# FyroxEngine/Fyrox

Measured on NVIDIA H100. Metric: nodes culled + verts skinned /sec, higher is better.
Workload: dtype f32

## Files before the change

fyrox_b200/csrc/fyx_kernels.cu:

```cuda
#include <cstdlib>
#include <cstring>

#include <cuda_fp16.h>

#include "fyx_internal.h"
#include "fyx_trs.cuh"

namespace fyx {

__device__ __forceinline__ float4 ld_stream(const float4 *p)
{
    float4 v;
    asm volatile("ld.global.nc.L1::no_allocate.v4.f32 {%0,%1,%2,%3}, [%4];"
                 : "=f"(v.x), "=f"(v.y), "=f"(v.z), "=f"(v.w)
                 : "l"(p));
    return v;
}
__device__ __forceinline__ float2 ld_stream(const float2 *p)
{
    float2 v;
    asm volatile("ld.global.nc.L1::no_allocate.v2.f32 {%0,%1}, [%2];" : "=f"(v.x), "=f"(v.y) : "l"(p));
    return v;
}
__device__ __forceinline__ uint4 ld_stream(const uint4 *p)
// ... 657 lines not shown
        bs_pre[r] = (b < b1) ? fa.bone_slot[b] : FYX_NONE;
        si_pre[r] = (b < b1 && fa.stale_idx) ? fa.stale_idx[b] : FYX_NONE;
    }
    const uint32_t nf = a.flags[slot];
    nf_out = nf;
    wx = a.wa[0][slot];
    wy = a.wa[1][slot];
    wz = a.wa[2][slot];
    if (!(nf & F_DIRTY)) return;
    float mnx = wx.x, mny = wy.x, mnz = wz.x, mxx = wx.y, mxy = wy.y, mxz = wz.y;
    uint32_t kmnx = 0, kmny = 0, kmnz = 0, kmxx = 0, kmxy = 0, kmxz = 0;
    auto add_bone = [&](const uint32_t b, const uint32_t bs, const uint32_t si) {
        if (bs == FYX_NONE) return;
        float px, py, pz;
        if (si != FYX_NONE) {
            const float4 o = fa.stale_pos[si];
            px = o.x; py = o.y; pz = o.z;
        } else {
            px = a.G[0][bs].w;
            py = a.G[1][bs].w;
            pz = a.G[2][bs].w;
        }
        const uint32_t key = b - b0 + 1u;
        if (px < mnx) { mnx = px; kmnx = key; }
        if (py < mny) { mny = py; kmny = key; }
        if (pz < mnz) { mnz = pz; kmnz = key; }
        if (px > mxx) { mxx = px; kmxx = key; }
        if (py > mxy) { mxy = py; kmxy = key; }
        if (pz > mxz) { mxz = pz; kmxz = key; }
    };
#pragma unroll
    for (int r = 0; r < 2; ++r) add_bone(b0 + lane + 32u * r, bs_pre[r], si_pre[r]);
    for (uint32_t b = b0 + lane + 64u; b < b1; b += 32)
        add_bone(b, fa.bone_slot[b], fa.stale_idx ? fa.stale_idx[b] : FYX_NONE);
#pragma unroll
    for (int o = 16; o > 0; o >>= 1) {
        fold_min(mnx, kmnx, __shfl_xor_sync(0xFFFFFFFFu, mnx, o), __shfl_xor_sync(0xFFFFFFFFu, kmnx, o));
        fold_min(mny, kmny, __shfl_xor_sync(0xFFFFFFFFu, mny, o), __shfl_xor_sync(0xFFFFFFFFu, kmny, o));
        fold_min(mnz, kmnz, __shfl_xor_sync(0xFFFFFFFFu, mnz, o), __shfl_xor_sync(0xFFFFFFFFu, kmnz, o));
        fold_max(mxx, kmxx, __shfl_xor_sync(0xFFFFFFFFu, mxx, o), __shfl_xor_sync(0xFFFFFFFFu, kmxx, o));
        fold_max(mxy, kmxy, __shfl_xor_sync(0xFFFFFFFFu, mxy, o), __shfl_xor_sync(0xFFFFFFFFu, kmxy, o));
        fold_max(mxz, kmxz, __shfl_xor_sync(0xFFFFFFFFu, mxz, o), __shfl_xor_sync(0xFFFFFFFFu, kmxz, o));
    }
    wx = make_float2(mnx, mxx);
    wy = make_float2(mny, mxy);
    wz = make_float2(mnz, mxz);
    if (lane == 0) {
        a.wa[0][slot] = wx;
        a.wa[1][slot] = wy;
        a.wa[2][slot] = wz;
    }
}

template <int NFT>
__global__ void __launch_bounds__(kBlock) k_fold_bones(const NodeArrays a, const FoldArrays fa, const CullParams cp)
{
    pdl_trigger();
    pdl_wait();
    constexpr int kWarps = kBlock / 32;
    __shared__ float2 s_box[3][kWarps];
    __shared__ uint32_t s_nf[kWarps];
    const uint32_t warp = threadIdx.x >> 5, lane = threadIdx.x & 31u;
    const uint32_t i = blockIdx.x * kWarps + warp;
    uint32_t nf = 0u;
    float2 wx = make_float2(0.f, 0.f), wy = wx, wz = wx;
    if (i < fa.n) fold_mesh(a, fa, i, lane, nf, wx, wy, wz);
    if (NFT < 0) return;
    if (lane == 0) {
        s_box[0][warp] = wx;
        s_box[1][warp] = wy;
        s_box[2][warp] = wz;
        s_nf[warp] = (i < fa.n) ? nf : 0u;
    }
    __syncthreads();
    if (warp != 0) return;
    uint32_t vis_bits = 0u, gi = 0u, slot = 0u;
    const uint32_t m = blockIdx.x * kWarps + lane;
    if (lane < kWarps && m < fa.n) {
        PackedConsts kc;
        kc.one = make_float2(cp.one, cp.one);
        kc.negzero = make_float2(cp.negzero, cp.negzero);
        slot = fa.node_slot[m];
        const float2 bx = s_box[0][lane], by = s_box[1][lane], bz = s_box[2][lane];
        vis_bits = cull_bits<(NFT > 0 ? NFT : 0)>(s_nf[lane], a.mask[slot], bx, by, bz, cp, kc, aabb_is_tame(bx, by, bz), 0xFFFFFFFFu);
        if (vis_bits) gi = a.gidx[slot];
    }
    compact_emit_warp(vis_bits, gi, slot, cp);
}

__global__ void __launch_bounds__(kBlock) k_snapshot_bones(const NodeArrays a, const uint32_t n_late, const uint32_t *late_slot,
                                                           float4 *stale_pos)
{
    const uint32_t e = blockIdx.x * kBlock + threadIdx.x;
    if (e >= n_late) return;
    const uint32_t s = late_slot[e];
    stale_pos[e] = make_float4(a.G[0][s].w, a.G[1][s].w, a.G[2][s].w, 0.0f);
}

__device__ __forceinline__ void palette_entry(const NodeArrays &a, const SkinArrays &sk, const uint32_t e)
{
    const uint32_t bs = sk.bone_slot[e];
    Affine P;
    if (bs != FYX_NONE) {
        Affine Gm, IB;
        Gm.r0 = a.G[0][bs];
        Gm.r1 = a.G[1][bs];
        Gm.r2 = a.G[2][bs];
        IB.r0 = ld_stream(sk.ib[0] + e);
        IB.r1 = ld_stream(sk.ib[1] + e);
        IB.r2 = ld_stream(sk.ib[2] + e);
        P = affine_mul(Gm, IB);
    } else {
        P = affine_identity();
    }
    float4 *o = reinterpret_cast<float4 *>(sk.palette + 16 * (size_t)e);
    o[0] = make_float4(P.r0.x, P.r1.x, P.r2.x, 0.0f);
    o[1] = make_float4(P.r0.y, P.r1.y, P.r2.y, 0.0f);
    o[2] = make_float4(P.r0.z, P.r1.z, P.r2.z, 0.0f);
    o[3] = make_float4(P.r0.w, P.r1.w, P.r2.w, 1.0f);
}

__global__ void __launch_bounds__(kBlock) k_palette(const NodeArrays a, const SkinArrays sk)
{
    pdl_trigger();
    pdl_wait();
    const uint32_t e = blockIdx.x * kBlock + threadIdx.x;
    if (e < sk.n_entries) palette_entry(a, sk, e);
}

__device__ __forceinline__ float2 lo2(const float4 v) { return make_float2(v.x, v.y); }
__device__ __forceinline__ float2 hi2(const float4 v) { return make_float2(v.z, v.w); }

template <int S, int LOG2C>
__device__ __forceinline__ void skin_fill_palette(float4 *s_pal, const float *palette, const uint32_t bone_off, const uint32_t n_bones)
{
    constexpr int C = 1 << LOG2C;
    constexpr int PL = S * C;
    for (uint32_t b = threadIdx.x; b < n_bones; b += kBlock) {
        const float4 *m = reinterpret_cast<const float4 *>(palette + 16 * (size_t)(bone_off + b));
        const float4 c0 = m[0], c1 = m[1], c2 = m[2], c3 = m[3];
        const float4 A = make_float4(c0.x, c0.y, c1.x, c1.y);
        const float4 B = make_float4(c2.x, c2.y, c3.x, c3.y);
        const float4 Z = make_float4(c0.z, c1.z, c2.z, c3.z);
#pragma unroll
        for (int c = 0; c < C; ++c) {
            s_pal[0 * PL + c * S + b] = A;
            s_pal[1 * PL + c * S + b] = B;
            s_pal[2 * PL + c * S + b] = Z;
        }
    }
}

template <int S, int LOG2C>
__device__ __forceinline__ void skin_quad(const float4 *s_pal, const uint32_t lane, const float4 x4, const float4 y4, const float4 z4,
                                          const float4 nx4, const float4 ny4, const float4 nz4, const float4 w0, const float4 w1,
                                          const float4 w2, const float4 w3, const uint4 iq, float4 *po, float4 *no,
                                          const PackedConsts kc)
{
    constexpr int C = 1 << LOG2C;
    constexpr int PL = S * C;
    const float px[4] = {x4.x, x4.y, x4.z, x4.w}, py[4] = {y4.x, y4.y, y4.z, y4.w}, pz[4] = {z4.x, z4.y, z4.z, z4.w};
    const float nx[4] = {nx4.x, nx4.y, nx4.z, nx4.w}, ny[4] = {ny4.x, ny4.y, ny4.z, ny4.w}, nz[4] = {nz4.x, nz4.y, nz4.z, nz4.w};
    const float wk4[4][4] = {{w0.x, w1.x, w2.x, w3.x}, {w0.y, w1.y, w2.y, w3.y}, {w0.z, w1.z, w2.z, w3.z}, {w0.w, w1.w, w2.w, w3.w}};
    const uint32_t iv[4] = {iq.x, iq.y, iq.z, iq.w};
    float ox[4], oy[4], oz[4], mx[4], my[4], mz[4];
#pragma unroll
    for (int v = 0; v < 4; ++v) {
        const float2 pxx = make_float2(px[v], px[v]), pyy = make_float2(py[v], py[v]), pzz = make_float2(pz[v], pz[v]);
        const float2 nxx = make_float2(nx[v], nx[v]), nyy = make_float2(ny[v], ny[v]), nzz = make_float2(nz[v], nz[v]);
        const float2 pnx = make_float2(px[v], nx[v]), pny = make_float2(py[v], ny[v]), pnz = make_float2(pz[v], nz[v]);
        float2 acc_p = make_float2(0.0f, 0.0f), acc_n = make_float2(0.0f, 0.0f), acc_z = make_float2(0.0f, 0.0f);
        const float *wk = wk4[v];
#pragma unroll
        for (int k = 0; k < 4; ++k) {
            const uint32_t bone = (iv[v] >> (8 * k)) & 0xFFu;
            const float4 *row = s_pal + (((lane - bone) & (uint32_t)(C - 1)) * S + bone);
            const float4 A = row[0], B = row[PL], Z = row[2 * PL];
            const float2 ww = make_float2(wk[k], wk[k]);
            const float2 t = add2(add2(add2(mul2(lo2(A), pxx, kc), mul2(hi2(A), pyy, kc), kc), mul2(lo2(B), pzz, kc), kc), hi2(B), kc);
            acc_p = add2(acc_p, mul2(t, ww, kc), kc);
            const float2 r = add2(add2(mul2(lo2(A), nxx, kc), mul2(hi2(A), nyy, kc), kc), mul2(lo2(B), nzz, kc), kc);
            acc_n = add2(acc_n, mul2(r, ww, kc), kc);
            float2 z = add2(add2(mul2(pnx, make_float2(Z.x, Z.x), kc), mul2(pny, make_float2(Z.y, Z.y), kc), kc), mul2(pnz, make_float2(Z.z, Z.z), kc), kc);
            z.x = FYX_ADD(z.x, Z.w);
            acc_z = add2(acc_z, mul2(z, ww, kc), kc);
        }
        ox[v] = acc_p.x; oy[v] = acc_p.y; oz[v] = acc_z.x;
        mx[v] = acc_n.x; my[v] = acc_n.y; mz[v] = acc_z.y;
    }
    st_stream(po + 0, make_float4(ox[0], oy[0], oz[0], ox[1]));
    st_stream(po + 1, make_float4(oy[1], oz[1], ox[2], oy[2]));
    st_stream(po + 2, make_float4(oz[2], ox[3], oy[3], oz[3]));
    st_stream(no + 0, make_float4(mx[0], my[0], mz[0], mx[1]));
    st_stream(no + 1, make_float4(my[1], mz[1], mx[2], my[2]));
    st_stream(no + 2, make_float4(mz[2], mx[3], my[3], mz[3]));
}

template <int S, int LOG2C>
__device__ __forceinline__ void skin_pair(const float4 *s_pal, const uint32_t lane, const float2 x2, const float2 y2, const float2 z2, const float2 nx2,
                                          const float2 ny2, const float2 nz2, const float2 w0, const float2 w1, const float2 w2, const float2 w3,
                                          const uint2 iq, float2 *po, float2 *no, const PackedConsts kc)
{
    constexpr int C = 1 << LOG2C;
    constexpr int PL = S * C;
    const float px[2] = {x2.x, x2.y}, py[2] = {y2.x, y2.y}, pz[2] = {z2.x, z2.y};
    const float nx[2] = {nx2.x, nx2.y}, ny[2] = {ny2.x, ny2.y}, nz[2] = {nz2.x, nz2.y};
    const float wk2[2][4] = {{w0.x, w1.x, w2.x, w3.x}, {w0.y, w1.y, w2.y, w3.y}};
    const uint32_t iv[2] = {iq.x, iq.y};
    float ox[2], oy[2], oz[2], mx[2], my[2], mz[2];
#pragma unroll
    for (int v = 0; v < 2; ++v) {
        const float2 pxx = make_float2(px[v], px[v]), pyy = make_float2(py[v], py[v]), pzz = make_float2(pz[v], pz[v]);
        const float2 nxx = make_float2(nx[v], nx[v]), nyy = make_float2(ny[v], ny[v]), nzz = make_float2(nz[v], nz[v]);
        const float2 pnx = make_float2(px[v], nx[v]), pny = make_float2(py[v], ny[v]), pnz = make_float2(pz[v], nz[v]);
        float2 acc_p = make_float2(0.0f, 0.0f), acc_n = make_float2(0.0f, 0.0f), acc_z = make_float2(0.0f, 0.0f);
        const float *wk = wk2[v];
#pragma unroll
        for (int k = 0; k < 4; ++k) {
            const uint32_t bone = (iv[v] >> (8 * k)) & 0xFFu;
            const float4 *row = s_pal + (((lane - bone) & (uint32_t)(C - 1)) * S + bone);
            const float4 A = row[0], B = row[PL], Z = row[2 * PL];
            const float2 ww = make_float2(wk[k], wk[k]);
            const float2 t = add2(add2(add2(mul2(lo2(A), pxx, kc), mul2(hi2(A), pyy, kc), kc), mul2(lo2(B), pzz, kc), kc), hi2(B), kc);
            acc_p = add2(acc_p, mul2(t, ww, kc), kc);
            const float2 r = add2(add2(mul2(lo2(A), nxx, kc), mul2(hi2(A), nyy, kc), kc), mul2(lo2(B), nzz, kc), kc);
            acc_n = add2(acc_n, mul2(r, ww, kc), kc);
            float2 z = add2(add2(mul2(pnx, make_float2(Z.x, Z.x), kc), mul2(pny, make_float2(Z.y, Z.y), kc), kc), mul2(pnz, make_float2(Z.z, Z.z), kc), kc);
            z.x = FYX_ADD(z.x, Z.w);
            acc_z = add2(acc_z, mul2(z, ww, kc), kc);
        }
        ox[v] = acc_p.x; oy[v] = acc_p.y; oz[v] = acc_z.x;
        mx[v] = acc_n.x; my[v] = acc_n.y; mz[v] = acc_z.y;
    }
    st_stream(po + 0, make_float2(ox[0], oy[0]));
    st_stream(po + 1, make_float2(oz[0], ox[1]));
    st_stream(po + 2, make_float2(oy[1], oz[1]));
    st_stream(no + 0, make_float2(mx[0], my[0]));
    st_stream(no + 1, make_float2(mz[0], mx[1]));
    st_stream(no + 2, make_float2(my[1], mz[1]));
}

template <int S, int LOG2C, int MINB>
__global__ void __launch_bounds__(kBlock, MINB) k_skin2(const SkinArrays sk, const SkinTile *__restrict__ tiles, const uint32_t n_tiles, const float one,
                                                      const float negzero)
{
    extern __shared__ float4 smem[];
    float4 *const s_pal = smem;
    PackedConsts kc;
    kc.one = make_float2(one, one);
    kc.negzero = make_float2(negzero, negzero);
    const SkinTile T = tiles[blockIdx.x];
    pdl_wait();
    skin_fill_palette<S, LOG2C>(s_pal, sk.palette, T.bone_off, T.n_bones);
    __syncthreads();
    const uint32_t lane = threadIdx.x & 31u;
    for (uint32_t h = threadIdx.x; h < 2u * T.n_quads; h += kBlock) {
        const size_t quad = (size_t)T.quad_start + (h >> 1);
        const float2 *row = reinterpret_cast<const float2 *>(sk.vblk + (quad >> 5) * kVblkStride + (quad & 31)) + (h & 1u);
        const float2 x2 = ld_stream(row + 0 * 64), y2 = ld_stream(row + 1 * 64), z2 = ld_stream(row + 2 * 64);
        const float2 nx2 = ld_stream(row + 3 * 64), ny2 = ld_stream(row + 4 * 64), nz2 = ld_stream(row + 5 * 64);
        const float2 w0 = ld_stream(row + 6 * 64), w1 = ld_stream(row + 7 * 64), w2 = ld_stream(row + 8 * 64), w3 = ld_stream(row + 9 * 64);
        const float2 iqf = ld_stream(row + 10 * 64);
        const uint2 iq = make_uint2(__float_as_uint(iqf.x), __float_as_uint(iqf.y));
        const size_t pair = 2 * quad + (h & 1u);
        skin_pair<S, LOG2C>(s_pal, lane, x2, y2, z2, nx2, ny2, nz2, w0, w1, w2, w3, iq, reinterpret_cast<float2 *>(sk.opos) + 3 * pair,
                            reinterpret_cast<float2 *>(sk.onrm) + 3 * pair, kc);
    }
}

__device__ __forceinline__ void bs_axpy(float4 &v, const uint2 h, const float w)
{
    const __half2 a = *reinterpret_cast<const __half2 *>(&h.x), b = *reinterpret_cast<const __half2 *>(&h.y);
    const float2 fa = __half22float2(a), fb = __half22float2(b);
    v.x = FYX_ADD(v.x, FYX_MUL(fa.x, w));
    v.y = FYX_ADD(v.y, FYX_MUL(fa.y, w));
    v.z = FYX_ADD(v.z, FYX_MUL(fb.x, w));
    v.w = FYX_ADD(v.w, FYX_MUL(fb.y, w));
}

__device__ __forceinline__ void apply_blend_shapes(const SkinArrays &sk, const SkinTile &T, const uint32_t q, float4 &x4, float4 &y4, float4 &z4,
                                                   float4 &nx4, float4 &ny4, float4 &nz4)
{
    const uint32_t e = T.local_quad0 + q;
    const uint2 *r0 = sk.bs + ((size_t)T.bs_off + (e >> 5)) * kBsBlockU2 + (e & 31u);
    const size_t shape_stride = (size_t)T.bs_blocks * kBsBlockU2;
    for (uint32_t sidx = 0; sidx < T.n_shapes; ++sidx) {
        const float w = sk.bs_w[T.w_off + sidx];
        const uint2 *r = r0 + sidx * shape_stride;
        const uint2 hx = r[0 * 32], hy = r[1 * 32], hz = r[2 * 32], hnx = r[3 * 32], hny = r[4 * 32], hnz = r[5 * 32];
        bs_axpy(x4, hx, w);
        bs_axpy(y4, hy, w);
        bs_axpy(z4, hz, w);
        bs_axpy(nx4, hnx, w);
        bs_axpy(ny4, hny, w);
        bs_axpy(nz4, hnz, w);
    }
}

__global__ void __launch_bounds__(kBlock) k_bs_layout(const uint32_t n_verts, const uint32_t n_shapes, const uint32_t layer_stride,
                                                      const uint16_t *rec, uint16_t *dst, const uint32_t bs_blocks)
{
    const uint64_t t = (uint64_t)blockIdx.x * kBlock + threadIdx.x;
    const uint64_t per_shape = (uint64_t)bs_blocks * 128;
    if (t >= per_shape * n_shapes) return;
    const uint32_t sidx = (uint32_t)(t / per_shape), v = (uint32_t)(t % per_shape);
    uint16_t h[6] = {0, 0, 0, 0, 0, 0};
    if (v < n_verts) {
        const uint16_t *r = rec + ((size_t)sidx * layer_stride + v) * 9;
        for (int k = 0; k < 6; ++k) h[k] = r[k];
    }
    uint16_t *blk = dst + ((size_t)sidx * bs_blocks + (v >> 7)) * (kBsBlockU2 * 4);
    const uint32_t g = (v >> 2) & 31u, j = v & 3u;
    for (int k = 0; k < 6; ++k) blk[(k * 32 + g) * 4 + j] = h[k];
}

void launch_bs_layout(cudaStream_t s, uint32_t n_verts, uint32_t n_shapes, uint32_t layer_stride, const uint16_t *d_records, uint2 *d_dst, uint32_t bs_blocks)
{
    if (!n_shapes || !bs_blocks) return;
    k_bs_layout<<<(unsigned)(((uint64_t)bs_blocks * 128 * n_shapes + kBlock - 1) / kBlock), kBlock, 0, s>>>(n_verts, n_shapes, layer_stride, d_records,
                                                                                                        reinterpret_cast<uint16_t *>(d_dst), bs_blocks);
}

template <int S, int LOG2C, int MINB, bool BS>
__global__ void __launch_bounds__(kBlock, MINB) k_skin(const SkinArrays sk, const SkinTile *__restrict__ tiles, const uint32_t n_tiles,
                                                     const float one, const float negzero)
{
    extern __shared__ float4 smem[];
    float4 *const s_pal = smem;
    PackedConsts kc;
    kc.one = make_float2(one, one);
    kc.negzero = make_float2(negzero, negzero);
    const SkinTile T = tiles[blockIdx.x];
    pdl_wait();
    skin_fill_palette<S, LOG2C>(s_pal, sk.palette, T.bone_off, T.n_bones);
    __syncthreads();
    const uint32_t lane = threadIdx.x & 31u;
    for (uint32_t q = threadIdx.x; q < T.n_quads; q += kBlock) {
        const size_t quad = (size_t)T.quad_start + q;
        const float4 *row = sk.vblk + (quad >> 5) * kVblkStride + (quad & 31);
        float4 x4 = ld_stream(row + 0 * 32), y4 = ld_stream(row + 1 * 32), z4 = ld_stream(row + 2 * 32);
        float4 nx4 = ld_stream(row + 3 * 32), ny4 = ld_stream(row + 4 * 32), nz4 = ld_stream(row + 5 * 32);
        const float4 w0 = ld_stream(row + 6 * 32), w1 = ld_stream(row + 7 * 32), w2 = ld_stream(row + 8 * 32), w3 = ld_stream(row + 9 * 32);
        const uint4 iq = ld_stream(reinterpret_cast<const uint4 *>(row + 10 * 32));
        if (BS && T.n_shapes) apply_blend_shapes(sk, T, q, x4, y4, z4, nx4, ny4, nz4);
        skin_quad<S, LOG2C>(s_pal, lane, x4, y4, z4, nx4, ny4, nz4, w0, w1, w2, w3, iq, reinterpret_cast<float4 *>(sk.opos) + 3 * quad,
                            reinterpret_cast<float4 *>(sk.onrm) + 3 * quad, kc);
    }
}

constexpr uint32_t kVblkBytes = kVblkStride * sizeof(float4);

__device__ __forceinline__ uint32_t smem_u32(const void *p) { return (uint32_t)__cvta_generic_to_shared(p); }
__device__ __forceinline__ void mbar_init(const uint32_t bar, const uint32_t count)
{
    asm volatile("mbarrier.init.shared::cta.b64 [%0], %1;" ::"r"(bar), "r"(count) : "memory");
}
__device__ __forceinline__ void mbar_expect_tx(const uint32_t bar, const uint32_t bytes)
{
    asm volatile("mbarrier.arrive.expect_tx.shared::cta.b64 _, [%0], %1;" ::"r"(bar), "r"(bytes) : "memory");
}
__device__ __forceinline__ void mbar_wait(const uint32_t bar, const uint32_t parity)
{
    asm volatile(
        "{\n"
        ".reg .pred p;\n"
        "WAIT_%=:\n"
        "mbarrier.try_wait.parity.shared::cta.b64 p, [%0], %1;\n"
        "@p bra DONE_%=;\n"
        "bra WAIT_%=;\n"
        "DONE_%=:\n"
        "}\n" ::"r"(bar),
        "r"(parity)
        : "memory");
}
__device__ __forceinline__ void bulk_g2s(const uint32_t dst, const void *src, const uint32_t bytes, const uint32_t bar)
{
    asm volatile("cp.async.bulk.shared::cluster.global.mbarrier::complete_tx::bytes [%0], [%1], %2, [%3];" ::"r"(dst), "l"(src), "r"(bytes), "r"(bar)
                 : "memory");
}

template <int S, int LOG2C, int STAGES, int MINB>
__global__ void __launch_bounds__(kBlock, MINB) k_skin_tma(const SkinArrays sk, const SkinTile *__restrict__ tiles, const uint32_t n_tiles,
                                                         const float one, const float negzero)
{
    constexpr int C = 1 << LOG2C;
    constexpr int W = kBlock / 32;
    constexpr uint32_t kPalBytes = (3u * S * C * sizeof(float4) + 127u) & ~127u;
    extern __shared__ __align__(128) unsigned char smem_raw[];
    float4 *const s_pal = reinterpret_cast<float4 *>(smem_raw);
    unsigned char *const ring = smem_raw + kPalBytes;
    uint64_t *const bars = reinterpret_cast<uint64_t *>(ring + (size_t)W * STAGES * kVblkBytes);
    PackedConsts kc;
    kc.one = make_float2(one, one);
    kc.negzero = make_float2(negzero, negzero);
    const SkinTile T = tiles[blockIdx.x];
    const uint32_t lane = threadIdx.x & 31u, warp = threadIdx.x >> 5;
    const uint32_t b0 = T.quad_start >> 5, b1 = (T.quad_start + T.n_quads + 31u) >> 5;
    const uint32_t q_lo = T.quad_start, q_hi = T.quad_start + T.n_quads;
    unsigned char *const my_ring = ring + (size_t)warp * STAGES * kVblkBytes;
    const uint32_t my_bar = smem_u32(bars + warp * STAGES);
    if (lane == 0) {
#pragma unroll
        for (int st = 0; st < STAGES; ++st) mbar_init(my_bar + 8u * st, 1u);
        asm volatile("fence.mbarrier_init.release.cluster;" ::: "memory");
    }
    __syncwarp();
    if (lane == 0) {
#pragma unroll
        for (int st = 0; st < STAGES; ++st) {
            const uint32_t b = b0 + warp + (uint32_t)st * W;
            if (b < b1) {
                mbar_expect_tx(my_bar + 8u * st, kVblkBytes);
                bulk_g2s(smem_u32(my_ring + (size_t)st * kVblkBytes), sk.vblk + (size_t)b * kVblkStride, kVblkBytes, my_bar + 8u * st);
            }
        }
    }
    pdl_wait();
    skin_fill_palette<S, LOG2C>(s_pal, sk.palette, T.bone_off, T.n_bones);
    __syncthreads();
    uint32_t j = 0;
    for (uint32_t b = b0 + warp; b < b1; b += W, ++j) {
        const uint32_t st = j % STAGES, parity = (j / STAGES) & 1u;
        mbar_wait(my_bar + 8u * st, parity);
        const float4 *row = reinterpret_cast<const float4 *>(my_ring + (size_t)st * kVblkBytes) + lane;
        const size_t quad = ((size_t)b << 5) + lane;
        if (quad >= q_lo && quad < q_hi) {
            const float4 x4 = row[0 * 32], y4 = row[1 * 32], z4 = row[2 * 32];
            const float4 nx4 = row[3 * 32], ny4 = row[4 * 32], nz4 = row[5 * 32];
            const float4 w0 = row[6 * 32], w1 = row[7 * 32], w2 = row[8 * 32], w3 = row[9 * 32];
            const uint4 iq = *reinterpret_cast<const uint4 *>(row + 10 * 32);
            skin_quad<S, LOG2C>(s_pal, lane, x4, y4, z4, nx4, ny4, nz4, w0, w1, w2, w3, iq, reinterpret_cast<float4 *>(sk.opos) + 3 * quad,
                                reinterpret_cast<float4 *>(sk.onrm) + 3 * quad, kc);
        }
        __syncwarp();
        const uint32_t nb = b + (uint32_t)STAGES * W;
        if (lane == 0 && nb < b1) {
            mbar_expect_tx(my_bar + 8u * st, kVblkBytes);
            bulk_g2s(smem_u32(my_ring + (size_t)st * kVblkBytes), sk.vblk + (size_t)nb * kVblkStride, kVblkBytes, my_bar + 8u * st);
        }
    }
}

__device__ __forceinline__ uint32_t resolve_slot(const uint32_t *d_idx, uint32_t e, const uint32_t *slot_of_node,
                                                 uint32_t n_nodes)
{
    const uint32_t node = d_idx ? d_idx[e] : e;
    if (node >= n_nodes) return FYX_NONE;
    return slot_of_node[node];
}

__device__ __forceinline__ bool load_affine_rows(const float *m16, Affine &A)
{
    const float4 *c = reinterpret_cast<const float4 *>(m16);
    const float4 c0 = c[0], c1 = c[1], c2 = c[2], c3 = c[3];
    A.r0 = make_float4(c0.x, c1.x, c2.x, c3.x);
    A.r1 = make_float4(c0.y, c1.y, c2.y, c3.y);
    A.r2 = make_float4(c0.z, c1.z, c2.z, c3.z);
    const bool bottom = (__float_as_uint(c0.w) == 0u) & (__float_as_uint(c1.w) == 0u) & (__float_as_uint(c2.w) == 0u) &
                        (c3.w == 1.0f);
    return bottom & finite4(A.r0) & finite4(A.r1) & finite4(A.r2);
}

__global__ void __launch_bounds__(kBlock) k_scatter_locals(const NodeArrays a, const uint32_t count, const uint32_t *d_idx,
                                                           const float *d_m16, const uint32_t *slot_of_node,
                                                           const uint32_t n_nodes, uint32_t *d_err)
{
    const uint32_t e = blockIdx.x * kBlock + threadIdx.x;
    if (e >= count) return;
    const uint32_t slot = resolve_slot(d_idx, e, slot_of_node, n_nodes);
    if (slot == FYX_NONE) return;
    Affine A;
    if (!load_affine_rows(d_m16 + 16 * (size_t)e, A)) {
        atomicOr(d_err, E_NOT_AFFINE);
        return;
    }
    a.L[0][slot] = A.r0;
    a.L[1][slot] = A.r1;
    a.L[2][slot] = A.r2;
    atomicOr(a.flags + slot, F_DIRTY_SELF);
}

template <bool HAS_STATICS, bool ROT_ONLY>
__global__ void __launch_bounds__(kBlock) k_scatter_trs(const NodeArrays a, const uint32_t count, const uint32_t *d_idx,
                                                        const void *d_payload, fyx_trs *trs_by_slot,
                                                        const fyx_transform_statics *st_by_slot, const uint32_t *slot_of_node,
                                                        const uint32_t n_nodes, uint32_t *d_err)
{
    const uint32_t e = blockIdx.x * kBlock + threadIdx.x;
    if (e >= count) return;
    const uint32_t slot = resolve_slot(d_idx, e, slot_of_node, n_nodes);
    if (slot == FYX_NONE) return;
    fyx_trs t;
    if (ROT_ONLY) {
        t = trs_by_slot[slot];
        const float4 q = static_cast<const float4 *>(d_payload)[e];
        t.rotation[0] = q.x; t.rotation[1] = q.y; t.rotation[2] = q.z; t.rotation[3] = q.w;
    } else {
        t = static_cast<const fyx_trs *>(d_payload)[e];
    }
// ... 232 lines not shown
    case 32: launch_pdl(KERNEL<NF, 32>, __VA_ARGS__); break;                     \
    case 34: launch_pdl(KERNEL<NF, 34>, __VA_ARGS__); break;                     \
    case 36: launch_pdl(KERNEL<NF, 36>, __VA_ARGS__); break;                     \
    case 38: launch_pdl(KERNEL<NF, 38>, __VA_ARGS__); break;                     \
    case 52: launch_pdl(KERNEL<NF, 52>, __VA_ARGS__); break;                     \
    default: launch_pdl(KERNEL<NF, 54>, __VA_ARGS__); break;                     \
    }

void launch_update_level(cudaStream_t s, const NodeArrays &a, uint32_t lo, uint32_t hi, bool update_all, const CullParams *cull)
{
    if (hi <= lo) return;
    if (cull) {
        const unsigned g = grid_for(hi - lo);
        const uint32_t ua = update_all ? 1u : 0u;
        int var = (cull_variant(cull->nf) & 3) | ((update_all && (cull_variant(cull->nf) & 4)) ? 4 : 0);
        if (cull_variant(cull->nf) & 8) var = (var & 5) | 8;
        if ((cull_variant(cull->nf) & 16) && update_all)
            var = (cull_variant(cull->nf) & 8) ? 28 : ((cull_variant(cull->nf) & 1) ? 21 : 20);
        if (cull_variant(cull->nf) & 32)
            var = 32 | (cull_variant(cull->nf) & 2) | (update_all ? ((cull_variant(cull->nf) & 16) ? 20 : (cull_variant(cull->nf) & 4)) : 0);
        switch (cull->nf) {
        case 1: FYX_DISPATCH_VAR(k_update_level, 1, var, g, kBlock, 0, s, a, lo, hi, ua, *cull); break;
        case 2: FYX_DISPATCH_VAR(k_update_level, 2, var, g, kBlock, 0, s, a, lo, hi, ua, *cull); break;
        case 3: FYX_DISPATCH_VAR(k_update_level, 3, var, g, kBlock, 0, s, a, lo, hi, ua, *cull); break;
        case 4: FYX_DISPATCH_VAR(k_update_level, 4, var, g, kBlock, 0, s, a, lo, hi, ua, *cull); break;
        case 6: FYX_DISPATCH_VAR(k_update_level, 6, var, g, kBlock, 0, s, a, lo, hi, ua, *cull); break;
        default: FYX_DISPATCH_VAR(k_update_level, 0, var, g, kBlock, 0, s, a, lo, hi, ua, *cull); break;
        }
    } else {
        CullParams none;
        none.nf = 0;
        if (update_all && (cull_variant(0) & 16)) launch_pdl(k_update_level<-1, 20>, grid_for(hi - lo), kBlock, 0, s, a, lo, hi, 1u, none);
        else if (update_all && (cull_variant(0) & 4)) launch_pdl(k_update_level<-1, 4>, grid_for(hi - lo), kBlock, 0, s, a, lo, hi, 1u, none);
        else launch_pdl(k_update_level<-1, 0>, grid_for(hi - lo), kBlock, 0, s, a, lo, hi, update_all ? 1u : 0u, none);
    }
}

template <int NFT> static void launch_subforest_t(cudaStream_t s, const NodeArrays &a, const SubforestPlan &sf, bool ua, const CullParams &cp)
{
    const bool defer = NFT >= 0 && cull_defers_compaction(cp.nf);
    if (ua && defer) launch_pdl(k_update_subforest<NFT, true, true>, sf.n_ctas, kBlock, 0, s, a, sf.rng, (int)sf.n_levels, 1u, cp);
    else if (ua) launch_pdl(k_update_subforest<NFT, true, false>, sf.n_ctas, kBlock, 0, s, a, sf.rng, (int)sf.n_levels, 1u, cp);
    else if (defer) launch_pdl(k_update_subforest<NFT, false, true>, sf.n_ctas, kBlock, 0, s, a, sf.rng, (int)sf.n_levels, 0u, cp);
    else launch_pdl(k_update_subforest<NFT, false, false>, sf.n_ctas, kBlock, 0, s, a, sf.rng, (int)sf.n_levels, 0u, cp);
}

void launch_update_subforest(cudaStream_t s, const NodeArrays &a, const SubforestPlan &sf, bool update_all, const CullParams *cull)
{
    if (!sf.n_ctas || !sf.n_levels) return;
    if (!cull) {
        CullParams none;
        none.nf = 0;
        launch_subforest_t<-1>(s, a, sf, update_all, none);
        return;
    }
    switch (cull->nf) {
    case 1: launch_subforest_t<1>(s, a, sf, update_all, *cull); break;
    case 6: launch_subforest_t<6>(s, a, sf, update_all, *cull); break;
    default: launch_subforest_t<0>(s, a, sf, update_all, *cull); break;
    }
}

void launch_compact_vis(cudaStream_t s, const NodeArrays &a, const CullParams &cp)
{
    if (!a.cap || !cp.nf) return;
    launch_pdl(k_compact_vis, grid_for(((uint64_t)a.cap + 7) / 8), kBlock, 0, s, a, cp);
}

__global__ void __launch_bounds__(kBlock) k_select_probes(const NodeArrays a, const LodParams obs, uint32_t *best)
{
    const uint32_t slot = blockIdx.x * kBlock + threadIdx.x;
    if (slot >= a.cap) return;
    const uint32_t nf = a.flags[slot];
    if ((nf & (FYX_NODE_ALIVE | FYX_NODE_REFLECTION_PROBE)) != (FYX_NODE_ALIVE | FYX_NODE_REFLECTION_PROBE)) return;
    const float2 wx = a.wa[0][slot], wy = a.wa[1][slot], wz = a.wa[2][slot];
    const uint32_t gi = a.gidx[slot];
    for (int f = 0; f < obs.nf; ++f) {
        const float px = obs.ox[f], py = obs.oy[f], pz = obs.oz[f];
        if (px >= wx.x && px <= wx.y && py >= wy.x && py <= wy.y && pz >= wz.x && pz <= wz.y) atomicMax(best + f, gi + 1u);
    }
}

void launch_select_probes(cudaStream_t s, const NodeArrays &a, const LodParams &obs, uint32_t *best)
{
    if (!a.cap || !obs.nf) return;
    k_select_probes<<<grid_for(a.cap), kBlock, 0, s>>>(a, obs, best);
}

void launch_cull_lights(cudaStream_t s, const NodeArrays &a, const CullParams &cp, uint32_t *const *d_out_ptrs, uint32_t *counts)
{
    if (!a.cap) return;
    k_cull_lights<<<grid_for(a.cap), kBlock, 0, s>>>(a, cp, d_out_ptrs, counts);
}

template <int NF> static void launch_cull_t(cudaStream_t s, unsigned g, int var, const NodeArrays &a, const CullParams &cp, const uint32_t *lodp, uint32_t lo,
                                            uint32_t hi, uint32_t *prune)
{
    switch (var) {
    case 0: k_cull<NF, 0><<<g, kBlock, 0, s>>>(a, cp, lodp, lo, hi, prune); break;
    case 1: k_cull<NF, 1><<<g, kBlock, 0, s>>>(a, cp, lodp, lo, hi, prune); break;
    case 2: k_cull<NF, 2><<<g, kBlock, 0, s>>>(a, cp, lodp, lo, hi, prune); break;
    case 3: k_cull<NF, 3><<<g, kBlock, 0, s>>>(a, cp, lodp, lo, hi, prune); break;
    case 32: k_cull<NF, 32><<<g, kBlock, 0, s>>>(a, cp, lodp, lo, hi, prune); break;
    default: k_cull<NF, 34><<<g, kBlock, 0, s>>>(a, cp, lodp, lo, hi, prune); break;
    }
}

void launch_cull_range(cudaStream_t s, const NodeArrays &a, const CullParams &cp, const uint32_t *lodp, uint32_t lo, uint32_t hi, uint32_t *prune)
{
    if (hi <= lo) return;
    const unsigned g = grid_for(hi - lo);
    const int var = (cull_variant(cp.nf) & 32) ? (32 | (cull_variant(cp.nf) & 2)) : (cull_variant(cp.nf) & 3);
    switch (cp.nf) {
    case 1: launch_cull_t<1>(s, g, var, a, cp, lodp, lo, hi, prune); break;
    case 2: launch_cull_t<2>(s, g, var, a, cp, lodp, lo, hi, prune); break;
    case 3: launch_cull_t<3>(s, g, var, a, cp, lodp, lo, hi, prune); break;
    case 4: launch_cull_t<4>(s, g, var, a, cp, lodp, lo, hi, prune); break;
    case 6: launch_cull_t<6>(s, g, var, a, cp, lodp, lo, hi, prune); break;
    default: launch_cull_t<0>(s, g, var, a, cp, lodp, lo, hi, prune); break;
    }
}

void launch_cull(cudaStream_t s, const NodeArrays &a, const CullParams &cp, const uint32_t *lodp) { launch_cull_range(s, a, cp, lodp, 0u, a.cap, nullptr); }

void launch_fold_bones(cudaStream_t s, const NodeArrays &a, const FoldArrays &fa, const CullParams *cull)
{
    if (!fa.n) return;
    const unsigned grid = grid_for((uint64_t)fa.n * 32);
    if (cull) {
        switch (cull->nf) {
        case 1: launch_pdl(k_fold_bones<1>, grid, kBlock, 0, s, a, fa, *cull); break;
        case 6: launch_pdl(k_fold_bones<6>, grid, kBlock, 0, s, a, fa, *cull); break;
        default: launch_pdl(k_fold_bones<0>, grid, kBlock, 0, s, a, fa, *cull); break;
        }
    } else {
        CullParams none;
        none.nf = 0;
        launch_pdl(k_fold_bones<-1>, grid, kBlock, 0, s, a, fa, none);
    }
}

void launch_snapshot_bones(cudaStream_t s, const NodeArrays &a, uint32_t n_late, const uint32_t *late_slot, float4 *stale_pos)
{
    if (!n_late) return;
    k_snapshot_bones<<<grid_for(n_late), kBlock, 0, s>>>(a, n_late, late_slot, stale_pos);
}

void launch_palette(cudaStream_t s, const NodeArrays &a, const SkinArrays &sk)
{
    if (!sk.n_entries) return;
    launch_pdl(k_palette, grid_for(sk.n_entries), kBlock, 0, s, a, sk);
}

template <int S, int LOG2C, int MINB, bool BS> static void launch_skin_t2(cudaStream_t s, const SkinArrays &sk, const SkinTile *tiles, uint32_t n_tiles)
{
    constexpr size_t smem_pal = (size_t)3 * S * (1 << LOG2C) * sizeof(float4);
    static bool init = false;
    if (!init) {
        cudaFuncSetAttribute(k_skin<S, LOG2C, MINB, BS>, cudaFuncAttributeMaxDynamicSharedMemorySize, (int)smem_pal);
        init = true;
    }
    launch_pdl(k_skin<S, LOG2C, MINB, BS>, n_tiles, kBlock, smem_pal, s, sk, tiles, n_tiles, 1.0f, -0.0f);
}
template <int S, int LOG2C, int MINB> static void launch_skin_t(cudaStream_t s, const SkinArrays &sk, const SkinTile *tiles, uint32_t n_tiles, bool bs)
{
    if (bs) launch_skin_t2<S, LOG2C, MINB, true>(s, sk, tiles, n_tiles);
    else launch_skin_t2<S, LOG2C, MINB, false>(s, sk, tiles, n_tiles);
}

template <int S, int LOG2C, int STAGES, int MINB> static void launch_skin_tma_t(cudaStream_t s, const SkinArrays &sk, const SkinTile *tiles, uint32_t n_tiles)
{
    constexpr size_t pal = ((size_t)3 * S * (1 << LOG2C) * sizeof(float4) + 127) & ~size_t(127);
    constexpr size_t smem = pal + (size_t)(kBlock / 32) * STAGES * kVblkBytes + (size_t)(kBlock / 32) * STAGES * 8;
    static bool init = false;
    if (!init) {
        cudaFuncSetAttribute(k_skin_tma<S, LOG2C, STAGES, MINB>, cudaFuncAttributeMaxDynamicSharedMemorySize, (int)smem);
        init = true;
    }
    launch_pdl(k_skin_tma<S, LOG2C, STAGES, MINB>, n_tiles, kBlock, smem, s, sk, tiles, n_tiles, 1.0f, -0.0f);
}

template <int S, int LOG2C, int MINB> static void launch_skin2_t(cudaStream_t s, const SkinArrays &sk, const SkinTile *tiles, uint32_t n_tiles)
{
    constexpr size_t smem_pal = (size_t)3 * S * (1 << LOG2C) * sizeof(float4);
    static bool init = false;
    if (!init) {
        cudaFuncSetAttribute(k_skin2<S, LOG2C, MINB>, cudaFuncAttributeMaxDynamicSharedMemorySize, (int)smem_pal);
        init = true;
    }
    launch_pdl(k_skin2<S, LOG2C, MINB>, n_tiles, kBlock, smem_pal, s, sk, tiles, n_tiles, 1.0f, -0.0f);
}

static int skin_variant()
{
    static int v = [] {
        const char *e = getenv("FYX_SKIN_VARIANT");
        if (!e || !*e) return 0;
        if (!strcmp(e, "tma2")) return 2;
        if (!strcmp(e, "tma3")) return 3;
        if (!strcmp(e, "pair4")) return 14;
        if (!strcmp(e, "pair5")) return 15;
        if (!strcmp(e, "pair6")) return 16;
        return 0;
    }();
    return v;
}

void launch_skin(cudaStream_t s, const SkinArrays &sk, const SkinTile *tiles, uint32_t n_tiles, uint32_t max_bones, bool blend_shapes)
{
    if (!n_tiles) return;
    const int var = skin_variant();
    if (var && max_bones <= 64 && !blend_shapes) {
        if (var == 2) launch_skin_tma_t<65, 2, 2, 2>(s, sk, tiles, n_tiles);
        else if (var == 3) launch_skin_tma_t<65, 3, 3, 1>(s, sk, tiles, n_tiles);
        else if (var == 14) launch_skin2_t<65, 3, 4>(s, sk, tiles, n_tiles);
        else if (var == 15) launch_skin2_t<65, 3, 5>(s, sk, tiles, n_tiles);
        else launch_skin2_t<65, 3, 6>(s, sk, tiles, n_tiles);
        return;
    }
    if (max_bones <= 64) {
        launch_skin_t<65, 3, 3>(s, sk, tiles, n_tiles, blend_shapes);
    } else if (max_bones <= 128) {
        launch_skin_t<129, 3, 3>(s, sk, tiles, n_tiles, blend_shapes);
    } else {
        launch_skin_t<257, 2, 3>(s, sk, tiles, n_tiles, blend_shapes);
    }
}

void launch_scatter_locals(cudaStream_t s, const NodeArrays &a, uint32_t count, const uint32_t *d_idx, const float *d_m16,
                           const uint32_t *slot_of_node, uint32_t n_nodes, uint32_t *d_err)
{
    if (!count) return;
    k_scatter_locals<<<grid_for(count), kBlock, 0, s>>>(a, count, d_idx, d_m16, slot_of_node, n_nodes, d_err);
}

void launch_scatter_trs(cudaStream_t s, const NodeArrays &a, uint32_t count, const uint32_t *d_idx, const void *d_payload, bool rot_only,
                        fyx_trs *trs_by_slot, const fyx_transform_statics *st, const uint32_t *slot_of_node, uint32_t n_nodes,
                        uint32_t *d_err)
{
    if (!count) return;
    const unsigned g = grid_for(count);
    if (rot_only) {
        if (st) k_scatter_trs<true, true><<<g, kBlock, 0, s>>>(a, count, d_idx, d_payload, trs_by_slot, st, slot_of_node, n_nodes, d_err);
        else k_scatter_trs<false, true><<<g, kBlock, 0, s>>>(a, count, d_idx, d_payload, trs_by_slot, st, slot_of_node, n_nodes, d_err);
    } else {
        if (st) k_scatter_trs<true, false><<<g, kBlock, 0, s>>>(a, count, d_idx, d_payload, trs_by_slot, st, slot_of_node, n_nodes, d_err);
        else k_scatter_trs<false, false><<<g, kBlock, 0, s>>>(a, count, d_idx, d_payload, trs_by_slot, st, slot_of_node, n_nodes, d_err);
    }
}

__global__ void __launch_bounds__(kBlock) k_fill_identity_trs(fyx_trs *t, const uint32_t n)
{
    const uint32_t e = blockIdx.x * kBlock + threadIdx.x;
    if (e >= n) return;
    fyx_trs r;
    r.position[0] = r.position[1] = r.position[2] = 0.f;
    r.rotation[0] = r.rotation[1] = r.rotation[2] = 0.f;
    r.rotation[3] = 1.f;
    r.scale[0] = r.scale[1] = r.scale[2] = 1.f;
    t[e] = r;
}

void launch_fill_identity_trs(cudaStream_t s, fyx_trs *t, uint32_t n)
{
    if (!n) return;
    k_fill_identity_trs<<<grid_for(n), kBlock, 0, s>>>(t, n);
}

void launch_scatter_statics(cudaStream_t s, const NodeArrays &a, uint32_t count, const uint32_t *d_idx, const fyx_transform_statics *d_in,
                            fyx_transform_statics *st, const uint32_t *slot_of_node, uint32_t n_nodes)
{
    if (!count) return;
    k_scatter_statics<<<grid_for(count), kBlock, 0, s>>>(a, count, d_idx, d_in, st, slot_of_node, n_nodes);
}

void launch_fill_default_statics(cudaStream_t s, fyx_transform_statics *st, uint32_t n)
{
    if (!n) return;
    k_fill_default_statics<<<grid_for(n), kBlock, 0, s>>>(st, n);
}

void launch_scatter_u32(cudaStream_t s, uint32_t *dst_col, uint32_t count, const uint32_t *d_idx,
                        const uint32_t *d_val, const uint32_t *slot_of_node, uint32_t n_nodes, int mode)
{
    if (!count) return;
    k_scatter_u32<<<grid_for(count), kBlock, 0, s>>>(dst_col, count, d_idx, d_val, slot_of_node, n_nodes, mode);
}

void launch_scatter_aabbs(cudaStream_t s, const NodeArrays &a, uint32_t count, const uint32_t *d_idx, const float *d_aabb6,
                          const uint32_t *slot_of_node, uint32_t n_nodes)
{
    if (!count) return;
    k_scatter_aabbs<<<grid_for(count), kBlock, 0, s>>>(a, count, d_idx, d_aabb6, slot_of_node, n_nodes);
}

void launch_gather_globals(cudaStream_t s, const NodeArrays &a, uint32_t count, const uint32_t *d_idx,
                           const uint32_t *slot_of_node, uint32_t n_nodes, float *d_out)
{
    if (!count) return;
    k_gather_globals<<<grid_for(count), kBlock, 0, s>>>(a, count, d_idx, slot_of_node, n_nodes, d_out);
}

void launch_gather_aabbs(cudaStream_t s, const NodeArrays &a, uint32_t count, const uint32_t *d_idx,
                         const uint32_t *slot_of_node, uint32_t n_nodes, float *d_out6)
{
    if (!count) return;
    k_gather_aabbs<<<grid_for(count), kBlock, 0, s>>>(a, count, d_idx, slot_of_node, n_nodes, d_out6);
}

void launch_gather_flags(cudaStream_t s, const NodeArrays &a, uint32_t count, const uint32_t *d_idx,
                         const uint32_t *slot_of_node, uint32_t n_nodes, uint32_t *d_out)
{
    if (!count) return;
    k_gather_flags<<<grid_for(count), kBlock, 0, s>>>(a, count, d_idx, slot_of_node, n_nodes, d_out);
}

void launch_deinterleave(cudaStream_t s, uint32_t n_verts, const unsigned char *d_bytes, fyx_vertex_layout layout,
                         uint32_t n_bones, float4 *vblk, uint64_t first_vertex, uint32_t *d_err)
{
    const uint32_t n_padded = (n_verts + 3u) & ~3u;
    if (!n_padded) return;
    k_deinterleave<<<grid_for(n_padded), kBlock, 0, s>>>(n_verts, n_padded, d_bytes, layout, n_bones, vblk, first_vertex, d_err);
}

void launch_ib_rows(cudaStream_t s, uint32_t n, const float *d_m16, float4 *r0, float4 *r1, float4 *r2, uint32_t *d_err)
{
    if (!n) return;
    k_ib_rows<<<grid_for(n), kBlock, 0, s>>>(n, d_m16, r0, r1, r2, d_err);
}

void launch_or_u32(cudaStream_t s, uint32_t *p, uint32_t bits) { k_or_u32<<<1, 1, 0, s>>>(p, bits); }

void launch_permute_words(cudaStream_t s, void *dst, const void *src, const uint32_t *map, uint32_t n, uint32_t words, const PermuteDefault &def)
{
    if (!n || !words) return;
    k_permute_words<<<grid_for((uint64_t)n * words), kBlock, 0, s>>>(static_cast<uint32_t *>(dst), static_cast<const uint32_t *>(src), map, n, words, def);
}

void launch_compact_gathered(cudaStream_t s, const uint32_t *pad, uint32_t maxc, const uint32_t *counts_all, int nranks, int f,
                             uint32_t *dst)
{
    if (!maxc || nranks <= 0) return;
    k_compact_gathered<<<grid_for((uint64_t)maxc * nranks), kBlock, 0, s>>>(pad, maxc, counts_all, nranks, f, dst);
}

}
```

Baseline: 32.31 billion.

## Stage skin output stores through shared memory and prefetch vertex blocks via cp.async

Result: faster. 37.73 billion (median of 6 runs) (+16.8%).

```diff
diff --git a/fyrox_b200/csrc/fyx_kernels.cu b/fyrox_b200/csrc/fyx_kernels.cu
--- a/fyrox_b200/csrc/fyx_kernels.cu
+++ b/fyrox_b200/csrc/fyx_kernels.cu
@@ -833,10 +833,10 @@
 }
 
 template <int S, int LOG2C>
-__device__ __forceinline__ void skin_quad(const float4 *s_pal, const uint32_t lane, const float4 x4, const float4 y4, const float4 z4,
-                                          const float4 nx4, const float4 ny4, const float4 nz4, const float4 w0, const float4 w1,
-                                          const float4 w2, const float4 w3, const uint4 iq, float4 *po, float4 *no,
-                                          const PackedConsts kc)
+__device__ __forceinline__ void skin_quad_regs(const float4 *s_pal, const uint32_t lane, const float4 x4, const float4 y4, const float4 z4,
+                                               const float4 nx4, const float4 ny4, const float4 nz4, const float4 w0, const float4 w1,
+                                               const float4 w2, const float4 w3, const uint4 iq, float4 (&po)[3], float4 (&no)[3],
+                                               const PackedConsts kc)
 {
     constexpr int C = 1 << LOG2C;
     constexpr int PL = S * C;
@@ -869,12 +869,26 @@
         ox[v] = acc_p.x; oy[v] = acc_p.y; oz[v] = acc_z.x;
         mx[v] = acc_n.x; my[v] = acc_n.y; mz[v] = acc_z.y;
     }
-    st_stream(po + 0, make_float4(ox[0], oy[0], oz[0], ox[1]));
-    st_stream(po + 1, make_float4(oy[1], oz[1], ox[2], oy[2]));
-    st_stream(po + 2, make_float4(oz[2], ox[3], oy[3], oz[3]));
-    st_stream(no + 0, make_float4(mx[0], my[0], mz[0], mx[1]));
-    st_stream(no + 1, make_float4(my[1], mz[1], mx[2], my[2]));
-    st_stream(no + 2, make_float4(mz[2], mx[3], my[3], mz[3]));
+    po[0] = make_float4(ox[0], oy[0], oz[0], ox[1]);
+    po[1] = make_float4(oy[1], oz[1], ox[2], oy[2]);
+    po[2] = make_float4(oz[2], ox[3], oy[3], oz[3]);
+    no[0] = make_float4(mx[0], my[0], mz[0], mx[1]);
+    no[1] = make_float4(my[1], mz[1], mx[2], my[2]);
+    no[2] = make_float4(mz[2], mx[3], my[3], mz[3]);
+}
+
+template <int S, int LOG2C>
+__device__ __forceinline__ void skin_quad(const float4 *s_pal, const uint32_t lane, const float4 x4, const float4 y4, const float4 z4,
+                                          const float4 nx4, const float4 ny4, const float4 nz4, const float4 w0, const float4 w1,
+                                          const float4 w2, const float4 w3, const uint4 iq, float4 *po, float4 *no,
+                                          const PackedConsts kc)
+{
+    float4 p[3], n[3];
+    skin_quad_regs<S, LOG2C>(s_pal, lane, x4, y4, z4, nx4, ny4, nz4, w0, w1, w2, w3, iq, p, n, kc);
+#pragma unroll
+    for (int j = 0; j < 3; ++j) st_stream(po + j, p[j]);
+#pragma unroll
+    for (int j = 0; j < 3; ++j) st_stream(no + j, n[j]);
 }
 
 template <int S, int LOG2C>
@@ -1002,30 +1016,104 @@
                                                                                                         reinterpret_cast<uint16_t *>(d_dst), bs_blocks);
 }
 
-template <int S, int LOG2C, int MINB, bool BS>
+__device__ __forceinline__ void store_lines(float4 *stage, const uint32_t lane, const bool valid, const float4 (&p)[3], const float4 (&n)[3],
+                                            float4 *po, float4 *no, const uint32_t n_f4)
+{
+    if (valid) {
+#pragma unroll
+        for (int j = 0; j < 3; ++j) {
+            stage[3 * lane + j] = p[j];
+            stage[96 + 3 * lane + j] = n[j];
+        }
+    }
+    __syncwarp();
+#pragma unroll
+    for (int j = 0; j < 3; ++j) {
+        const uint32_t i = lane + 32u * j;
+        if (i < n_f4) {
+            st_stream(po + i, stage[i]);
+            st_stream(no + i, stage[96 + i]);
+        }
+    }
+    __syncwarp();
+}
+
+__device__ __forceinline__ void cp_async16(float4 *dst, const float4 *src)
+{
+    asm volatile("cp.async.cg.shared.global [%0], [%1], 16;" ::"r"((uint32_t)__cvta_generic_to_shared(dst)), "l"(src) : "memory");
+}
+__device__ __forceinline__ void cp_async_commit() { asm volatile("cp.async.commit_group;" ::: "memory"); }
+__device__ __forceinline__ void cp_async_wait_all() { asm volatile("cp.async.wait_group 0;" ::: "memory"); }
+
+constexpr int kSkinStageF4 = 2 * 96;
+constexpr int kSkinRingF4 = kVblkRows * 32;
+template <int S, int LOG2C, bool PREFETCH> constexpr size_t skin_smem_bytes()
+{
+    return sizeof(float4) * ((size_t)3 * S * (1 << LOG2C) + (kBlock / 32) * (kSkinStageF4 + (PREFETCH ? kSkinRingF4 : 0)));
+}
+
+template <int S, int LOG2C, int MINB, bool BS, bool PREFETCH>
 __global__ void __launch_bounds__(kBlock, MINB) k_skin(const SkinArrays sk, const SkinTile *__restrict__ tiles, const uint32_t n_tiles,
                                                      const float one, const float negzero)
 {
+    constexpr int PAL = 3 * S * (1 << LOG2C);
     extern __shared__ float4 smem[];
     float4 *const s_pal = smem;
     PackedConsts kc;
     kc.one = make_float2(one, one);
     kc.negzero = make_float2(negzero, negzero);
     const SkinTile T = tiles[blockIdx.x];
+    const uint32_t lane = threadIdx.x & 31u, warp = threadIdx.x >> 5;
+    float4 *const stage = smem + PAL + warp * kSkinStageF4;
+    float4 *const ring = smem + PAL + (kBlock / 32) * kSkinStageF4 + warp * kSkinRingF4 + lane;
+    const uint32_t zero = __float_as_uint(negzero) << 1;
+    auto prefetch = [&](const uint32_t q, const uint32_t dep) {
+        if (q < T.n_quads) {
+            const size_t quad = (size_t)T.quad_start + q;
+            const float4 *row = sk.vblk + (quad >> 5) * kVblkStride + (quad & 31);
+#pragma unroll
+            for (int r = 0; r < kVblkRows; ++r) cp_async16(ring + r * 32 + dep, row + r * 32);
+        }
+        cp_async_commit();
+    };
+    if (PREFETCH) prefetch(threadIdx.x, 0);
     pdl_wait();
     skin_fill_palette<S, LOG2C>(s_pal, sk.palette, T.bone_off, T.n_bones);
     __syncthreads();
-    const uint32_t lane = threadIdx.x & 31u;
-    for (uint32_t q = threadIdx.x; q < T.n_quads; q += kBlock) {
+    for (uint32_t q0 = warp * 32; q0 < T.n_quads; q0 += kBlock) {
+        const uint32_t q = q0 + lane;
+        const bool valid = q < T.n_quads;
         const size_t quad = (size_t)T.quad_start + q;
-        const float4 *row = sk.vblk + (quad >> 5) * kVblkStride + (quad & 31);
-        float4 x4 = ld_stream(row + 0 * 32), y4 = ld_stream(row + 1 * 32), z4 = ld_stream(row + 2 * 32);
-        float4 nx4 = ld_stream(row + 3 * 32), ny4 = ld_stream(row + 4 * 32), nz4 = ld_stream(row + 5 * 32);
-        const float4 w0 = ld_stream(row + 6 * 32), w1 = ld_stream(row + 7 * 32), w2 = ld_stream(row + 8 * 32), w3 = ld_stream(row + 9 * 32);
-        const uint4 iq = ld_stream(reinterpret_cast<const uint4 *>(row + 10 * 32));
-        if (BS && T.n_shapes) apply_blend_shapes(sk, T, q, x4, y4, z4, nx4, ny4, nz4);
-        skin_quad<S, LOG2C>(s_pal, lane, x4, y4, z4, nx4, ny4, nz4, w0, w1, w2, w3, iq, reinterpret_cast<float4 *>(sk.opos) + 3 * quad,
-                            reinterpret_cast<float4 *>(sk.onrm) + 3 * quad, kc);
+        float4 x4, y4, z4, nx4, ny4, nz4, w0, w1, w2, w3;
+        uint4 iq;
+        if (PREFETCH) {
+            cp_async_wait_all();
+            if (valid) {
+                x4 = ring[0 * 32]; y4 = ring[1 * 32]; z4 = ring[2 * 32];
+                nx4 = ring[3 * 32]; ny4 = ring[4 * 32]; nz4 = ring[5 * 32];
+                w0 = ring[6 * 32]; w1 = ring[7 * 32]; w2 = ring[8 * 32]; w3 = ring[9 * 32];
+                iq = *reinterpret_cast<const uint4 *>(ring + 10 * 32);
+            }
+            const uint32_t dep = valid ? ((__float_as_uint(x4.x) ^ __float_as_uint(y4.x) ^ __float_as_uint(z4.x) ^ __float_as_uint(nx4.x) ^
+                                           __float_as_uint(ny4.x) ^ __float_as_uint(nz4.x) ^ __float_as_uint(w0.x) ^ __float_as_uint(w1.x) ^
+                                           __float_as_uint(w2.x) ^ __float_as_uint(w3.x) ^ iq.x) & zero)
+                                       : 0u;
+            prefetch(q + kBlock, dep);
+        } else if (valid) {
+            const float4 *row = sk.vblk + (quad >> 5) * kVblkStride + (quad & 31);
+            x4 = ld_stream(row + 0 * 32); y4 = ld_stream(row + 1 * 32); z4 = ld_stream(row + 2 * 32);
+            nx4 = ld_stream(row + 3 * 32); ny4 = ld_stream(row + 4 * 32); nz4 = ld_stream(row + 5 * 32);
+            w0 = ld_stream(row + 6 * 32); w1 = ld_stream(row + 7 * 32); w2 = ld_stream(row + 8 * 32); w3 = ld_stream(row + 9 * 32);
+            iq = ld_stream(reinterpret_cast<const uint4 *>(row + 10 * 32));
+        }
+        float4 p[3], n[3];
+        if (valid) {
+            if (BS && T.n_shapes) apply_blend_shapes(sk, T, q, x4, y4, z4, nx4, ny4, nz4);
+            skin_quad_regs<S, LOG2C>(s_pal, lane, x4, y4, z4, nx4, ny4, nz4, w0, w1, w2, w3, iq, p, n, kc);
+        }
+        const size_t f0 = 3 * ((size_t)T.quad_start + q0);
+        store_lines(stage, lane, valid, p, n, reinterpret_cast<float4 *>(sk.opos) + f0, reinterpret_cast<float4 *>(sk.onrm) + f0,
+                    3u * min(32u, T.n_quads - q0));
     }
 }
 
@@ -1564,20 +1652,22 @@
     launch_pdl(k_palette, grid_for(sk.n_entries), kBlock, 0, s, a, sk);
 }
 
-template <int S, int LOG2C, int MINB, bool BS> static void launch_skin_t2(cudaStream_t s, const SkinArrays &sk, const SkinTile *tiles, uint32_t n_tiles)
-{
-    constexpr size_t smem_pal = (size_t)3 * S * (1 << LOG2C) * sizeof(float4);
+template <int S, int LOG2C, int MINB, bool BS, bool PREFETCH>
+static void launch_skin_t2(cudaStream_t s, const SkinArrays &sk, const SkinTile *tiles, uint32_t n_tiles)
+{
+    constexpr size_t smem = skin_smem_bytes<S, LOG2C, PREFETCH>();
     static bool init = false;
     if (!init) {
-        cudaFuncSetAttribute(k_skin<S, LOG2C, MINB, BS>, cudaFuncAttributeMaxDynamicSharedMemorySize, (int)smem_pal);
+        cudaFuncSetAttribute(k_skin<S, LOG2C, MINB, BS, PREFETCH>, cudaFuncAttributeMaxDynamicSharedMemorySize, (int)smem);
         init = true;
     }
-    launch_pdl(k_skin<S, LOG2C, MINB, BS>, n_tiles, kBlock, smem_pal, s, sk, tiles, n_tiles, 1.0f, -0.0f);
-}
-template <int S, int LOG2C, int MINB> static void launch_skin_t(cudaStream_t s, const SkinArrays &sk, const SkinTile *tiles, uint32_t n_tiles, bool bs)
-{
-    if (bs) launch_skin_t2<S, LOG2C, MINB, true>(s, sk, tiles, n_tiles);
-    else launch_skin_t2<S, LOG2C, MINB, false>(s, sk, tiles, n_tiles);
+    launch_pdl(k_skin<S, LOG2C, MINB, BS, PREFETCH>, n_tiles, kBlock, smem, s, sk, tiles, n_tiles, 1.0f, -0.0f);
+}
+template <int S, int LOG2C, int MINB, bool PREFETCH>
+static void launch_skin_t(cudaStream_t s, const SkinArrays &sk, const SkinTile *tiles, uint32_t n_tiles, bool bs)
+{
+    if (bs) launch_skin_t2<S, LOG2C, MINB, true, PREFETCH>(s, sk, tiles, n_tiles);
+    else launch_skin_t2<S, LOG2C, MINB, false, PREFETCH>(s, sk, tiles, n_tiles);
 }
 
 template <int S, int LOG2C, int STAGES, int MINB> static void launch_skin_tma_t(cudaStream_t s, const SkinArrays &sk, const SkinTile *tiles, uint32_t n_tiles)
@@ -1631,11 +1721,11 @@
         return;
     }
     if (max_bones <= 64) {
-        launch_skin_t<65, 3, 3>(s, sk, tiles, n_tiles, blend_shapes);
+        launch_skin_t<65, 3, 2, true>(s, sk, tiles, n_tiles, blend_shapes);
     } else if (max_bones <= 128) {
-        launch_skin_t<129, 3, 3>(s, sk, tiles, n_tiles, blend_shapes);
+        launch_skin_t<129, 3, 3, false>(s, sk, tiles, n_tiles, blend_shapes);
     } else {
-        launch_skin_t<257, 2, 3>(s, sk, tiles, n_tiles, blend_shapes);
+        launch_skin_t<257, 2, 3, false>(s, sk, tiles, n_tiles, blend_shapes);
     }
 }
 
```
